# MiloniAtal/gato-python

Hardware: AMD Instinct MI355X
Metric: PCG iterations/s (higher is better)
Workload: dtype f64; 1 GPU; iiwa_14_7_k50_f64; STATE_SIZE=14, CONTROL_SIZE=7, KNOT_POINTS=50, max_iters=100, pcg_kernel=resident (one workgroup, mixed 2/1 rows per lane), pcg_workgroups=1, pcg_threads=512

## Files before the change

gato_python_amd/csrc/gato_assembly.hip:

```cpp
#include "gato_common.h"
#include "gato_gj.h"

namespace gato {
namespace {

constexpr int WAVE = 64;

template <typename T, int S, int C>
__global__ void add_rho_kernel(const T *__restrict__ G_in, T rho, T *__restrict__ Gd, size_t n_per_sys, int B)
{
    constexpr int SS = S * S, CC = C * C;
    const size_t total = n_per_sys * B;
    for (size_t i = (size_t)blockIdx.x * blockDim.x + threadIdx.x; i < total; i += (size_t)gridDim.x * blockDim.x) {
        const size_t w = (i % n_per_sys) % (SS + CC);
        const bool diag = w < SS ? (w % (S + 1) == 0) : ((w - SS) % (C + 1) == 0);
        Gd[i] = G_in[i] + (diag ? rho : (T)0);
    }
}

__device__ __forceinline__ void wave_sync() { __syncthreads(); }

template <typename T>
__device__ __forceinline__ void copy_in(T *dst, const T *__restrict__ src, int n, int lane)
{
// ... 306 lines not shown
    static constexpr int n = S + C, SS = S * S, CC = C * C, SC = S * C;
    static constexpr int Q = 0;
    static constexpr int R = Q + 3 * SS;
    static constexpr int AB = R + 3 * CC;
    static constexpr int PHI = AB + 2 * (SS + SC);
    static constexpr int BR = PHI + 2 * SS;
    static constexpr int TH = BR + 2 * SC;
    static constexpr int TT = TH + 2 * SS;
    static constexpr int VQ = TT + 2 * SS;
    static constexpr int VV = VQ + 2 * S + C;
    static constexpr int ELEMS = (VV + 3 * S + 3) / 4 * 4;
    static constexpr int PTR_G = 3 * n + 1, PTR_C = 2 * S + 1;
    static constexpr size_t BYTES = sizeof(T) * ELEMS + sizeof(int) * (PTR_G + PTR_C);
};

__device__ __forceinline__ int row_of_entry(const int *ptr, int nrows, int e)
{
    int lo = 0, hi = nrows;
    while (hi - lo > 1) {
        const int mid = (lo + hi) >> 1;
        if (ptr[mid] <= e) lo = mid; else hi = mid;
    }
    return lo;
}

template <typename T, int S, int C, int NT>
__global__ __launch_bounds__(NT, (GatherWaves<T, S>::v)) void gather_kernel(const int *__restrict__ G_row, const int *__restrict__ G_col,
                                                    const T *__restrict__ G_val, const int *__restrict__ C_row,
                                                    const int *__restrict__ C_col, const T *__restrict__ C_val, int K, T rho,
                                                    T *__restrict__ Gd, T *__restrict__ Cd, T *__restrict__ Ginv, BatchStride bs)
{
    constexpr int n = S + C, SS = S * S, CC = C * C, SC = S * C, ABS = SS + SC;
    static_assert(NT % WAVE == 0, "whole waves");
    __shared__ T blk[SS + CC + ABS];
    __shared__ int sPtrG[n + 1], sPtrC[S + 1];
    constexpr int NSLOT = SS + CC + ABS;
    __shared__ unsigned smask[(NSLOT + 31) / 32];
    __shared__ int sown[NSLOT];
    __shared__ int s_coll;
    T *sQ = blk, *sR = blk + SS, *sAB = blk + SS + CC;
    const int tid = threadIdx.x, lane = tid & 63, wave = tid >> 6;
    G_val += blockIdx.y * bs.nnzG; C_val += blockIdx.y * bs.nnzC;
    Gd += blockIdx.y * bs.g; Cd += blockIdx.y * bs.c;
    if (Ginv) Ginv += blockIdx.y * bs.g;
    for (int k = bs.k_lo + blockIdx.x; k < bs.k_hi; k += gridDim.x) {
        const bool last = k == K - 1;
// ... 52 lines not shown
                for (int t = tid; t < nG + nC; t += NT) {
                    const int colv = t < nG ? G_col[eG0 + t] : C_col[eC0 + (t - nG)];
                    const T valv = t < nG ? G_val[eG0 + t] : C_val[eC0 + (t - nG)];
                    T v;
                    const int sl = slot_of(t, colv, valv, v);
                    if (sl < 0) continue;
                    if (pass == 0) atomicMax(&sown[sl], t);
                    else if (sown[sl] == t) blk[sl] = v;
                }
                __syncthreads();
            }
        }
        __syncthreads();
        const size_t gk = (size_t)k * (SS + CC);
        for (int i = tid; i < SS + (last ? 0 : CC); i += NT) Gd[gk + i] = blk[i];
        if (!last) for (int i = tid; i < ABS; i += NT) Cd[(size_t)k * ABS + i] = sAB[i];
        if (Ginv) {
            if (wave == 0) invert_to<T, S>(sQ, Ginv + gk, lane, (T)1);
            if (wave == (NT > WAVE ? 1 : 0) && !last) invert_to<T, C>(sR, Ginv + gk + SS, lane, (T)1);
        }
    }
}

template <typename T, int S, int C, int NT>
__global__ __launch_bounds__(NT) void assemble_kernel(AsmArgs a, int K, BatchStride bs)
{
    typedef AsmLds<T, S, C> L;
    constexpr int n = S + C, SS = S * S, CC = C * C, SC = S * C, NW = NT / WAVE, ABS = SS + SC;
    static_assert(NW >= 6, "six inversions run side by side");
    constexpr int TILES = ((S + 15) / 16) * ((S + 15) / 16);
    extern __shared__ __align__(16) unsigned char lds_raw[];
    T *lds = (T *)lds_raw;
    T *sQ = lds + L::Q, *sR = lds + L::R, *sAB = lds + L::AB, *sPhi = lds + L::PHI, *sBR = lds + L::BR;
    T *sTh = lds + L::TH, *sT = lds + L::TT, *sq = lds + L::VQ, *sv = lds + L::VV;
    int *sPtrG = (int *)(lds + L::ELEMS), *sPtrC = sPtrG + L::PTR_G;
    constexpr int NSLOT = 3 * SS + 3 * CC + 2 * ABS;
    __shared__ unsigned smask[(NSLOT + 31) / 32];
    __shared__ int sown[NSLOT];
    __shared__ int s_coll;
    const int tid = threadIdx.x, lane = tid & 63, wave = tid >> 6;
    const int sys = blockIdx.y;
    const T *g = (const T *)a.g + sys * bs.n, *c = (const T *)a.c + sys * bs.sk;
    T *Gd = (T *)a.Gd + sys * bs.g, *Cd = (T *)a.Cd + sys * bs.c, *Ginv = (T *)a.Ginv + sys * bs.g;
    T *Sbd = (T *)a.Sbd + sys * bs.bd, *Pbd = (T *)a.Pbd + sys * bs.bd, *gamma = (T *)a.gamma + sys * bs.sk;
    const T rho = (T)a.rho;
    T *const iS = (T *)a.imgS, *const iP = (T *)a.imgP;
    const size_t ild = (size_t)a.img_ld;
    auto imS = [&](int kk, int b, int r, int cc, T v) { if (iS) iS[(size_t)(b * S + cc) * ild + (size_t)kk * S + r] = v; };
    auto imP = [&](int kk, int b, int r, int cc, T v) { if (iP) iP[(size_t)(b * S + cc) * ild + (size_t)kk * S + r] = v; };
    T *sQk = sQ + 2 * SS, *sRk = sR + 2 * CC, *sQm = sQ + SS, *sRm = sR + CC, *sQmm = sQ, *sRmm = sR;
    T *sA1 = sAB + ABS, *sB1 = sA1 + SS, *sA0 = sAB, *sB0 = sAB + SS;
    T *sPhi1 = sPhi + SS, *sPhi0 = sPhi, *sBR1 = sBR + SC, *sBR0 = sBR, *sTh1 = sTh + SS, *sTh0 = sTh;
    int n_stamp = 0;
    auto stamp = [&]() {
        if (a.stamps && blockIdx.x == (K > 2 ? 2 : 0) && sys == 0 && tid == 0) a.stamps[n_stamp++] = __builtin_amdgcn_s_memrealtime();
    };
    stamp();

    for (int k = blockIdx.x; k < K; k += gridDim.x) {
        const bool first = k == 0, last = k == K - 1;
        const bool full0 = k >= 2;
        const size_t gk = (size_t)k * (SS + CC);
        const size_t cm = first ? 0 : (size_t)(k - 1) * ABS;
        T *Sk = Sbd + (size_t)k * 3 * SS, *Pk = Pbd + (size_t)k * 3 * SS;
        static_assert(2 * S + C <= NT && S <= NT - 2 * WAVE, "one element of g and of c per thread");
        const int n_gq = first ? S : n + S;
        const int i_cq = first ? tid : tid - 2 * WAVE;
        const T gq = tid < n_gq ? g[(first ? 0 : (size_t)(k - 1) * n) + tid] : (T)0;
        const T cq = i_cq >= 0 && i_cq < S ? c[(size_t)k * S + i_cq] : (T)0;
        __syncthreads();
        if (a.mode == 0) {
            const T *G_val = (const T *)a.G_val + sys * bs.nnzG, *C_val = (const T *)a.C_val + sys * bs.nnzC;
            const int r0 = (k >= 2 ? k - 2 : 0) * n, nrG = k * n + (last ? S : n) - r0;
            const int c0 = (k >= 2 ? k - 1 : 1) * S, nrC = first ? 0 : (k + 1) * S - c0;
            static_assert(L::PTR_G <= NT && L::PTR_C <= NT, "one row pointer per thread");
            const int pG = tid <= nrG ? a.G_row[r0 + tid] : 0;
            const int pC = nrC && tid <= nrC ? a.C_row[c0 + tid] : 0;
            for (int i = tid; i < 3 * SS + 3 * CC + 2 * ABS; i += NT) lds[i] = (T)0;
            for (int i = tid; i < (NSLOT + 31) / 32; i += NT) smask[i] = 0u;
            if (tid == 0) s_coll = 0;
            if (tid <= nrG) sPtrG[tid] = pG;
            if (nrC && tid <= nrC) sPtrC[tid] = pC;
            __syncthreads();
            const int eG0 = sPtrG[0], nG = sPtrG[nrG] - eG0;
            const int eC0 = nrC ? sPtrC[0] : 0, nC = nrC ? sPtrC[nrC] - eC0 : 0;
            auto slot_of = [&](int t, int colv, T valv, T &v) -> int {
                if (t < nG) {
                    const int row = r0 + row_of_entry(sPtrG, nrG, eG0 + t);
                    const int knot = row / n, isr = row - knot * n, qi = knot - (k - 2);
                    const int isc = colv % n;
                    v = valv + (colv == row ? rho : (T)0);
                    if (isc < S) return isr < S ? L::Q + qi * SS + isc * S + isr : -1;
                    return isr >= S ? L::R + qi * CC + (isc - S) * C + (isr - S) : -1;
                }
                const int row = c0 + row_of_entry(sPtrC, nrC, eC0 + (t - nG));
                const int br = row / S - 1, i = row - (br + 1) * S;
                v = valv;
                return colv / n <= br ? L::AB + (br - (k - 2)) * ABS + (colv % n) * S + i : -1;
            };
            constexpr int U = 4;
            for (int t0 = tid; t0 < nG + nC; t0 += NT * U) {
                int col[U];
                T val[U];
#pragma unroll
                for (int u = 0; u < U; ++u) {
                    const int t = t0 + u * NT;
                    if (t < nG) { col[u] = a.G_col[eG0 + t]; val[u] = G_val[eG0 + t]; }
                    else if (t < nG + nC) { col[u] = a.C_col[eC0 + (t - nG)]; val[u] = C_val[eC0 + (t - nG)]; }
                }
#pragma unroll
                for (int u = 0; u < U; ++u) {
                    const int t = t0 + u * NT;
                    if (t < nG + nC) {
                        T v;
                        const int sl = slot_of(t, col[u], val[u], v);
                        if (sl >= 0) {
                            lds[sl] = v;
                            const unsigned bit = 1u << (sl & 31);
                            if (atomicOr(&smask[sl >> 5], bit) & bit) s_coll = 1;
                        }
                    }
                }
            }
            __syncthreads();
            if (s_coll) {
                for (int i = tid; i < NSLOT; i += NT) sown[i] = -1;
                __syncthreads();
                for (int pass = 0; pass < 2; ++pass) {
                    for (int t = tid; t < nG + nC; t += NT) {
                        const int colv = t < nG ? a.G_col[eG0 + t] : a.C_col[eC0 + (t - nG)];
                        const T valv = t < nG ? G_val[eG0 + t] : C_val[eC0 + (t - nG)];
                        T v;
                        const int sl = slot_of(t, colv, valv, v);
                        if (sl < 0) continue;
                        if (pass == 0) atomicMax(&sown[sl], t);
                        else if (sown[sl] == t) lds[sl] = v;
                    }
                    __syncthreads();
                }
            }
        } else {
            const T *Gin = a.mode == 2 ? (const T *)a.G_val + sys * bs.g : Gd;
            const T r2 = a.mode == 2 ? rho : (T)0;
#pragma unroll
            for (int qi = 0; qi < 3; ++qi) {
                const int knot = k - 2 + qi;
                if (knot < 0) continue;
                const size_t go = (size_t)knot * (SS + CC);
                for (int i = tid; i < SS; i += NT) sQ[qi * SS + i] = Gin[go + i] + ((i % (S + 1) == 0) ? r2 : (T)0);
                if (knot < K - 1)
                    for (int i = tid; i < CC; i += NT) sR[qi * CC + i] = Gin[go + SS + i] + ((i % (C + 1) == 0) ? r2 : (T)0);
                if (qi < 2 && knot < K - 1) copy_nt<NT>(sAB + qi * ABS, Cd + (size_t)knot * ABS, ABS, tid);
            }
        }
        if (tid < n_gq) sq[tid] = gq;
        __syncthreads();
        stamp();
        if (a.mode != 1) {
            for (int i = tid; i < SS; i += NT) Gd[gk + i] = sQk[i];
            if (!last) for (int i = tid; i < CC; i += NT) Gd[gk + SS + i] = sRk[i];
            if (a.mode == 0 && !first) for (int i = tid; i < ABS; i += NT) Cd[cm + i] = sA1[i];
        }
        if (first) for (int i = tid; i < SS; i += NT) { Pk[SS + i] = -sQk[i]; imP(0, 1, i % S, i / S, -sQk[i]); }
        if (k == 1) for (int i = tid; i < SS; i += NT) sTh0[i] = -sQm[i];
        __syncthreads();
        {
            T *mS = wave == 0 ? sQk : wave == 1 ? sQm : sQmm, *mC = wave == 5 ? sRk : wave == 2 ? sRm : sRmm;
            if (wave == 0 || (wave == 1 && !first) || (wave == 3 && full0)) invert_to<T, S>(mS, mS, lane, (T)1);
            else if ((wave == 5 && !last) || (wave == 2 && !first) || (wave == 4 && full0)) invert_to<T, C>(mC, mC, lane, (T)1);
        }
        __syncthreads();
        stamp();
        for (int i = tid; i < SS; i += NT) Ginv[gk + i] = sQk[i];
        if (!last) for (int i = tid; i < CC; i += NT) Ginv[gk + SS + i] = sRk[i];
        if (first) {
            if (wave == 0) mv<T, S, S>(sv, sQk, sq, lane);
            for (int i = tid; i < SS; i += NT) {
                Sk[i] = (T)0;
                Sk[SS + i] = -sQk[i];
// ... 170 lines not shown
    bs.stair_follows = d.stair_follows;
    if (!have_inverses) {
        const int nblk = (2 * (d.hi() - d.lo()) + 3) / 4;
        hipLaunchKernelGGL((invert_G_kernel<T, S, C>), dim3(nblk < 8192 ? nblk : 8192, d.B), dim3(256), 0, st, Gd, Ginv, d.K,
                           batch_stride(d));
        GATO_HIP_CHECK(hipGetLastError());
    }
    hipLaunchKernelGGL((schur_kernel<T, S, C>), dim3(knot_grid(d.hi() - d.lo()), d.B), dim3(WAVE), 0, st, Gd, Ginv, Cd, g, c, d.K,
                       Sbd, Pbd, gamma, bs);
    GATO_HIP_CHECK(hipGetLastError());
    return GATO_OK;
}

template <typename T, int S, int C>
int launch_assemble(const Dims &d, const AsmArgs &a, hipStream_t st)
{
    constexpr int NT = 512;
    typedef AsmLds<T, S, C> L;
    if (L::BYTES > 48 * 1024) {
        static bool attr_set[64] = {};
        int dev = 0;
        GATO_HIP_CHECK(hipGetDevice(&dev));
        if (dev < 0 || dev >= 64 || !attr_set[dev]) {
            GATO_HIP_CHECK(hipFuncSetAttribute((const void *)assemble_kernel<T, S, C, NT>,
                                               hipFuncAttributeMaxDynamicSharedMemorySize, (int)L::BYTES));
            if (dev >= 0 && dev < 64) attr_set[dev] = true;
        }
    }
    const int gx = d.K < (1 << 20) ? d.K : (1 << 20);
    hipLaunchKernelGGL((assemble_kernel<T, S, C, NT>), dim3(gx, d.B), dim3(NT), L::BYTES, st, a, d.K, batch_stride(d));
    GATO_HIP_CHECK(hipGetLastError());
    return GATO_OK;
}

template <typename T, int S, int C>
int launch_form_ss(const Dims &d, const T *Sbd, T *Pbd, hipStream_t st)
{
    hipLaunchKernelGGL((ss_kernel<T, S>), dim3(knot_grid(d.hi() - d.lo()), d.B), dim3(WAVE), 0, st, Sbd, Pbd, d.K, batch_stride(d));
    GATO_HIP_CHECK(hipGetLastError());
    return GATO_OK;
}

template <typename T, int S, int C>
int launch_point_jacobi(const Dims &d, const T *Sbd, T *Pbd, hipStream_t st)
{
    const size_t total = d.bd();
    const int blocks = (int)((total + 255) / 256 < 4096 ? (total + 255) / 256 : 4096);
    hipLaunchKernelGGL((point_jacobi_kernel<T, S>), dim3(blocks, d.B), dim3(256), 0, st, Sbd, Pbd, d.K, batch_stride(d));
    GATO_HIP_CHECK(hipGetLastError());
    return GATO_OK;
}

template <typename T, int S, int C>
// ... 37 lines not shown
```

gato_python_amd/csrc/gato_capi.hip:

```cpp
#include <cmath>
#include <cstdarg>
#include <cstdlib>
#include "gato_solver.h"

namespace gato {

static thread_local char g_err[512] = "";

void set_error(const char *fmt, ...)
{
    va_list ap;
    va_start(ap, fmt);
    vsnprintf(g_err, sizeof(g_err), fmt, ap);
    va_end(ap);
}

}

using namespace gato;

bool solver_usable(const gato_solver *s, const char *entry, const char *unsupported)
{
    if (!s) set_error("%s: null solver", entry);
    else if (s->cl.on || s->cl.local) set_error("%s: the solver is a cluster rank; sharded %s are not supported", entry, unsupported);
// ... 103 lines not shown
        return GATO_ENODEV;
    }
    GATO_HIP_CHECK(hipSetDevice(device));
    gato_solver *s = new gato_solver();
    memset(s, 0, sizeof(*s));
    s->d = Dims{S, C, K};
    s->d.B = B;
    s->dtype = dtype;
    s->device = device;
    s->esz = dtype == GATO_F32 ? 4 : 8;
    s->ops = ops;
    hipDeviceProp_t p;
    GATO_HIP_CHECK(hipGetDeviceProperties(&p, device));
    s->num_cus = p.multiProcessorCount;
    ops->pcg_plan(&s->plan);
    s->pcg_mode = GATO_PCG_AUTO;
    s->xcd_pack = -1;
    s->xcd_sel = -1;
    s->wave_pub = 1;
    s->dpp_rows = -1;
    s->pcg_semi = -1;
    s->timeout_ms = 2000;
    s->cluster_flat = 1;

    const Dims &d = s->d;
    const size_t e = s->esz;
    const int max_groups = 4096;
    size_t off = 0;
    auto take = [&](size_t bytes) { size_t o = off; off += align_up(bytes ? bytes : 8); return o; };
    const size_t o_status = take(64);
    const int slot_g = pcg_slot_granules(S, (int)e) > pcg_slot_granules_cg1(S, (int)e) ? pcg_slot_granules(S, (int)e)
                                                                                        : pcg_slot_granules_cg1(S, (int)e);
    const size_t o_slots = take((size_t)2 * 256 * slot_g * 8);
    s->slots_bytes = (size_t)2 * 256 * slot_g * 8;
    const size_t nb = (size_t)B;
    const size_t o_G = take(d.g_dense() * e * nb), o_C = take(d.c_dense() * e * nb), o_Gi = take(d.g_dense() * e * nb);
    const size_t o_S = take(d.bd() * e * nb), o_P = take(d.bd() * e * nb), o_gam = take(d.sk() * e * nb);
    const size_t o_lam = take(d.sk() * e * nb), o_dz = take(d.N() * e * nb);
    const size_t o_its = take(sizeof(int) * nb);
    const size_t o_vec = take(6 * d.sk() * e);
    const size_t o_part = take((size_t)4 * max_groups * e), o_scal = take(64 * 8), o_done = take(64);
    const size_t o_gh = take((size_t)8 * S * e);
    const size_t o_hist = take(sizeof(double) * (GATO_ETA_HIST_MAX + 1));
    const size_t o_xtab = take(sizeof(void *) * GATO_MAX_RANKS);
    const long long rows = (long long)K * S;
    const bool img = B == 1 && ((s->plan.pair_threads > 0 && rows <= 2ll * s->plan.pair_threads) || (s->plan.mixed_rows > 0 && rows <= s->plan.mixed_rows));
// ... 32 lines not shown
}

extern "C" int gato_solver_destroy(gato_solver *s)
{
    if (!s) return GATO_OK;
    (void)hipSetDevice(s->device);
    gato_cluster_destroy(s);
    if (s->ev_pcg0) (void)hipEventDestroy(s->ev_pcg0);
    if (s->ev_pcg1) (void)hipEventDestroy(s->ev_pcg1);
    if (s->ev_cal0) (void)hipEventDestroy(s->ev_cal0);
    if (s->ev_cal1) (void)hipEventDestroy(s->ev_cal1);
    for (int i = 0; i < 4; ++i)
        if (s->ev_stage[i]) (void)hipEventDestroy(s->ev_stage[i]);
    if (s->arena) (void)hipFree(s->arena);
    if (s->rhs_ws) (void)hipFree(s->rhs_ws);
    if (s->qp_ws) (void)hipFree(s->qp_ws);
    if (s->pol_ws) (void)hipFree(s->pol_ws);
    if (s->cross_ws) (void)hipFree(s->cross_ws);
    if (s->cross_rhs_ws) (void)hipFree(s->cross_rhs_ws);
    if (s->in_arena) (void)hipFree(s->in_arena);
    for (int i = 0; i < 2; ++i)
        if (s->host_ev[i]) (void)hipEventDestroy(s->host_ev[i]);
    if (s->pin) (void)hipHostFree(s->pin);
    delete s;
    return GATO_OK;
}

extern "C" void *gato_solver_buffer(gato_solver *s, int which)
{
    switch (which) {
        case 0: return s->G_dense;
        case 1: return s->C_dense;
        case 2: return s->Ginv;
        case 3: return s->Sbd;
        case 4: return s->Pbd;
        case 5: return s->gamma;
        case 6: return s->lambda;
        case 7: return s->dz;
        case 8: return s->iters;
        case 9: return (unsigned long long *)s->sw.scalars + 8;
        case 10: return s->eta_hist;
        case 11: return s->rhs_ws;
        case 12: return s->qp_pcg_total;
        case 13: case 14: case 15: case 16: {
            if (!s->cross_ws) return nullptr;
            const size_t e = s->esz, nb = (size_t)s->d.B;
            size_t off = 0;
            if (which > 13) off += align_up(s->d.g_dense() * e * nb);
            if (which > 14) off += align_up(s->d.c_dense() * e * nb);
            if (which > 15) off += align_up((size_t)(s->d.K - 1) * s->d.S * s->d.C * e * nb);
            return s->cross_ws + off;
        }
        default: return nullptr;
    }
}

extern "C" int gato_solver_set_option(gato_solver *s, const char *name, int value)
{
    if (!strcmp(name, "pcg_mode")) s->pcg_mode = value;
    else if (!strcmp(name, "pcg_threads")) s->pcg_threads = value;
    else if (!strcmp(name, "pcg_groups")) s->pcg_groups = value;
    else if (!strcmp(name, "asm_mode")) s->asm_mode = value;
    else if (!strcmp(name, "pcg_semi")) s->pcg_semi = value;
    else if (!strcmp(name, "pcg_epoch")) s->pcg_epoch = (unsigned)value;
    else if (!strcmp(name, "cluster_epoch")) s->cl.xepoch = (unsigned)value;
    else if (!strcmp(name, "stamp_asm")) s->stamp_asm = value;
    else if (!strcmp(name, "stamp_pcg")) s->stamp_pcg = value;
    else if (!strcmp(name, "ablate")) s->ablate = value;
    else if (!strcmp(name, "no_single_lds")) s->no_single_lds = value;
    else if (!strcmp(name, "no_pair")) s->no_pair = value;
    else if (!strcmp(name, "wave_pub")) s->wave_pub = value;
    else if (!strcmp(name, "dpp_rows")) s->dpp_rows = value;
    else if (!strcmp(name, "pcg_variant")) s->pcg_variant = value;
    else if (!strcmp(name, "record_eta")) s->record_eta = value;
    else if (!strcmp(name, "xcd_pack")) s->xcd_pack = value;
    else if (!strcmp(name, "xcd_sel")) s->xcd_sel = value < 0 ? -1 : (value & 7);
    else if (!strcmp(name, "true_warm_start")) s->true_warm_start = value;
    else if (!strcmp(name, "timeout_ms")) s->timeout_ms = value > 0 ? value : 2000;
    else if (!strcmp(name, "max_workgroups")) s->max_workgroups = value;
    else if (!strcmp(name, "no_fuse_dz")) s->no_fuse_dz = value;
    else if (!strcmp(name, "no_image")) s->no_image = value;
    else if (!strcmp(name, "qp_cross_unfused")) s->qp_cross_unfused = value;
    else if (!strcmp(name, "coop_launch")) s->coop_launch = value;
    else if (!strcmp(name, "cluster_flat")) s->cluster_flat = value;
    else if (!strcmp(name, "knot_lo") || !strcmp(name, "knot_hi")) {
        if (value < 0 || value > s->d.K) { set_error("%s = %d is outside [0, %d]", name, value, s->d.K); return GATO_EINVAL; }
        (name[5] == 'l' ? s->d.k_lo : s->d.k_hi) = value;
    }
    else if (!strcmp(name, "precon_mode")) {
// ... 28 lines not shown

extern "C" int gato_last_stage_ms(gato_solver *s, float *ms)
{
    if (!s->time_stages || !s->ev_stage[0]) { set_error("last_stage_ms: option time_stages is off"); return GATO_EINVAL; }
    GATO_HIP_CHECK(hipEventSynchronize(s->ev_stage[3]));
    for (int i = 0; i < 3; ++i) GATO_HIP_CHECK(hipEventElapsedTime(ms + i, s->ev_stage[i], s->ev_stage[i + 1]));
    return GATO_OK;
}

extern "C" int gato_solver_get_option(gato_solver *s, const char *name, int *value)
{
    if (!strcmp(name, "pcg_mode")) *value = s->pcg_mode;
    else if (!strcmp(name, "pcg_threads")) *value = s->pcg_threads;
    else if (!strcmp(name, "pcg_groups")) *value = s->pcg_groups;
    else if (!strcmp(name, "last_groups")) *value = s->last_groups;
    else if (!strcmp(name, "last_threads")) *value = s->last_threads;
    else if (!strcmp(name, "last_mode")) *value = s->last_mode;
    else if (!strcmp(name, "last_pair")) *value = s->last_pair;
    else if (!strcmp(name, "last_dpp")) *value = s->last_dpp;
    else if (!strcmp(name, "last_xcd_sel")) *value = s->last_xcd_sel;
    else if (!strcmp(name, "last_variant")) *value = s->last_variant;
    else if (!strcmp(name, "asm_mode")) *value = s->asm_mode;
    else if (!strcmp(name, "last_asm_fused")) *value = s->last_asm_fused;
    else if (!strcmp(name, "last_image")) *value = s->last_image;
    else if (!strcmp(name, "last_semi")) *value = s->last_semi;
    else if (!strcmp(name, "last_fallback")) *value = s->last_fallback;
    else if (!strcmp(name, "last_dz_fused")) *value = s->dz_fused;
    else if (!strcmp(name, "last_cluster_flat")) *value = s->cl.on ? s->cl.last_flat : 0;
    else if (!strcmp(name, "timeout_ms")) *value = s->timeout_ms;
    else if (!strcmp(name, "precon_mode")) *value = s->precon_mode;
    else if (!strcmp(name, "cluster_mem_kind")) *value = s->cl.on ? s->cl.mem_kind : -1;
    else if (!strcmp(name, "num_cus")) *value = s->num_cus;
    else if (!strcmp(name, "batch")) *value = s->d.B;
    else if (!strcmp(name, "rhs_reserved")) *value = s->rhs_R;
    else if (!strcmp(name, "assembly_valid")) *value = s->as.valid;
    else if (!strcmp(name, "assembly_gen")) *value = (int)s->as.gen;
    else if (!strcmp(name, "true_warm_start")) *value = s->true_warm_start;
    else if (!strcmp(name, "max_semi_knots"))
        *value = s->plan.semi_threads > 0 ? (s->plan.semi_threads / s->d.S + s->plan.semi_rows * s->plan.semi_threads / s->d.S) * (s->num_cus < 256 ? s->num_cus : 256) : 0;
    else if (!strcmp(name, "max_resident_knots")) *value = s->plan.max_knots_per_wg * (s->num_cus < 256 ? s->num_cus : 256);
    else { set_error("unknown option %s", name); return GATO_EINVAL; }
    return GATO_OK;
}

static bool owned(const gato_solver *s, const void *p)
{
    const char *q = (const char *)p;
// ... 43 lines not shown
```

gato_python_amd/csrc/gato_common.h:

```cpp
#pragma once
#include <hip/hip_runtime.h>

#include <cstddef>
#include <cstdint>
#include <cstdio>
#include <cstring>

#include "../../include/gato_hip.h"

#ifndef GATO_EXTRA_SHAPES
#define GATO_EXTRA_SHAPES(X)
#endif
#ifndef GATO_SHAPES
#define GATO_SHAPES(X) X(2, 1) X(14, 7) X(32, 16) X(4, 2) X(6, 3) X(12, 6) GATO_EXTRA_SHAPES(X)
#endif

#define GATO_MAX_RANKS 8

namespace gato {

void set_error(const char *fmt, ...);

__device__ __forceinline__ float fmaT(float a, float b, float c) { return __builtin_fmaf(a, b, c); }
__device__ __forceinline__ double fmaT(double a, double b, double c) { return __builtin_fma(a, b, c); }
// ... 176 lines not shown

struct PcgPlan {
    int max_threads;
    int max_knots_per_wg;
    int single_max_threads;
    int pair_threads;
    int mixed_rows, mixed_threads;
    int semi_threads;
    int semi_rows;
    int nores_threads;
    int nores_rows;
    int dpp_lanes;
};

template <typename T, int S, int C>
int launch_convert(const Dims &d, const int *G_row, const int *G_col, const T *G_val, const int *C_row,
                   const int *C_col, const T *C_val, T rho, T *Gd, T *Cd, T *Ginv ,
                   hipStream_t st);
template <typename T, int S, int C>
int launch_add_rho(const Dims &d, const T *G_in, T rho, T *Gd, hipStream_t st);
template <typename T, int S, int C>
int launch_form_schur(const Dims &d, const T *Gd, const T *Cd, const T *g, const T *c, T *Sbd, T *Pbd,
                      T *gamma, T *Ginv, bool have_inverses, hipStream_t st);
struct AsmArgs {
    int mode;
    const int *G_row, *G_col, *C_row, *C_col;
    const void *G_val, *C_val;
    double rho;
    const void *g, *c;
    void *Gd, *Cd, *Ginv, *Sbd, *Pbd, *gamma;
    void *imgS, *imgP;
    int img_ld;
    unsigned long long *stamps;
};
template <typename T, int S, int C>
int launch_assemble(const Dims &d, const AsmArgs &a, hipStream_t st);

template <typename T, int S, int C>
int launch_form_ss(const Dims &d, const T *Sbd, T *Pbd, hipStream_t st);
template <typename T, int S, int C>
int launch_point_jacobi(const Dims &d, const T *Sbd, T *Pbd, hipStream_t st);
template <typename T, int S, int C>
int launch_compute_dz(const Dims &d, const T *Ginv, const T *Cd, const T *g, const T *lambda, T *dz,
                      hipStream_t st);
template <typename T, int S, int C>
int launch_rhs_gamma(const Dims &d, int R, const T *Ginv, const T *Cd, const T *Sbd, const T *g, const T *c, T *gamma,
                     hipStream_t st);
template <typename T, int S, int C>
int launch_grad_blocks(const Dims &d, const T *dz, const T *lam, const T *a, const T *beta, T *Gbar, T *Cbar, hipStream_t st);
template <typename T, int S, int C>
int launch_grad_csr(const Dims &d, const int *G_row, const int *G_col, int nnzG, const int *C_row, const int *C_col, int nnzC,
                    const T *dz, const T *lam, const T *a, const T *beta, T *Gbar, T *Cbar, hipStream_t st);
#define GATO_QP_NSLOT 10
struct QpArgs {
    const void *G, *Cd, *g, *c, *lo, *hi;
    void *Gp;
// ... 234 lines not shown
```

gato_python_amd/csrc/gato_solve.hip:

```cpp
#include "gato_solver.h"

static int assemble(gato_solver *s, const AsmInput &in, const void *d_g, const void *d_c, double rho, hipStream_t st)
{
    int rc;
    const int mode = in.mode;
    s->d.k_lo = s->d.k_hi = 0;
    const long long knots = (long long)s->d.K * s->d.B;
    const bool stair = s->precon_mode == GATO_PRECON_STAIR;
    const bool fused = !in.have_inv && stair && (s->asm_mode == 2 || (s->asm_mode == 0 && knots <= 2ll * s->num_cus));
    s->last_asm_fused = fused;
    s->img_fresh = 0;
    s->as.valid = 0;
    s->as.img = 0;
    if (!fused) {
        if (in.have_inv) rc = GATO_OK;
        else if (mode == 0) {
            if (s->d.B > 1 && (s->d.nnzG <= 0 || s->d.nnzC <= 0)) return gato_convert(s, in.G_row, in.G_col, in.G_val, in.C_row, in.C_col, in.C_val, rho, s->G_dense, s->C_dense, st);
            rc = s->ops->convert(s->d, in.G_row, in.G_col, in.G_val, in.C_row, in.C_col, in.C_val, rho, s->G_dense, s->C_dense, s->Ginv, st);
        } else rc = s->ops->add_rho(s->d, in.G_val, rho, s->G_dense, st);
        if (rc) return rc;
        s->d.stair_follows = s->precon_mode == GATO_PRECON_STAIR;
        rc = s->ops->form_schur(s->d, s->G_dense, in.C_dense, d_g, d_c, s->Sbd, s->Pbd, s->gamma, s->Ginv, mode == 0 || in.have_inv, st);
        s->d.stair_follows = 0;
        if (rc) return rc;
        if (s->precon_mode == GATO_PRECON_BLOCK_JACOBI) return GATO_OK;
        if (s->precon_mode == GATO_PRECON_POINT_JACOBI) return s->ops->point_jacobi(s->d, s->Sbd, s->Pbd, st);
        return gato_form_ss(s, s->Sbd, s->Pbd, st);
    }
    if (mode == 0 && s->d.B > 1 && (s->d.nnzG <= 0 || s->d.nnzC <= 0)) {
        set_error("a batched solver needs the per-system nnz (gato_linsys_device_batched, or options batch_nnz_G / batch_nnz_C)");
        return GATO_EINVAL;
    }
    AsmArgs a;
    memset(&a, 0, sizeof(a));
    a.mode = mode;
    a.G_row = in.G_row; a.G_col = in.G_col; a.G_val = in.G_val; a.C_row = in.C_row; a.C_col = in.C_col; a.C_val = in.C_val;
    a.rho = rho; a.g = d_g; a.c = d_c;
    a.Gd = s->G_dense; a.Cd = const_cast<void *>(in.C_dense); a.Ginv = s->Ginv; a.Sbd = s->Sbd; a.Pbd = s->Pbd; a.gamma = s->gamma;
    a.stamps = s->stamp_asm ? (unsigned long long *)s->sw.scalars + 8 : nullptr;
    if (s->imgS && !s->no_image && s->d.B == 1) {
        a.imgS = s->imgS; a.imgP = s->imgP; a.img_ld = s->img_ld;
        s->img_fresh = 1;
        s->as.img = 1;
    }
    return s->ops->assemble(s->d, a, st);
}

int whole_solve(gato_solver *s, const PcgOpts &o, const AsmInput &in, const void *d_g, const void *d_c, double exit_tol,
                int max_iters, double rho, void *lam, void *dz, hipStream_t st)
{
    int rc;
    const bool ts = s->time_stages != 0 && !in.have_inv;
    if (ts) GATO_HIP_CHECK(hipEventRecord(s->ev_stage[0], st));
    if ((rc = assemble(s, in, d_g, d_c, rho, st))) return rc;
    if (ts) GATO_HIP_CHECK(hipEventRecord(s->ev_stage[1], st));
    s->lc = {1, s->Sbd, s->Pbd, s->gamma, in.C_dense, d_g, lam, dz, exit_tol, max_iters};
    s->fz = {s->Ginv, in.C_dense, d_g, dz};
    rc = pcg_systems(s, o, s->Sbd, s->Pbd, s->gamma, lam, exit_tol, max_iters, s->iters, st);
    s->fz = {nullptr, nullptr, nullptr, nullptr};
    s->img_fresh = 0;
    if (rc) return rc;
    if (ts) GATO_HIP_CHECK(hipEventRecord(s->ev_stage[2], st));
    if (!s->dz_fused && (rc = gato_compute_dz(s, s->Ginv, in.C_dense, d_g, lam, dz, st))) return rc;
    if (ts) GATO_HIP_CHECK(hipEventRecord(s->ev_stage[3], st));
    s->as = {1, in.C_dense, s->as.img, s->as.gen + 1};
    return GATO_OK;
}

// ... 184 lines not shown
```

gato_python_amd/csrc/gato_solver.h:

```cpp
#pragma once
#include <mutex>

#include "gato_common.h"

using namespace gato;

#define GATO_ETA_HIST_MAX 4096

struct gato_solver {
    Dims d;
    int dtype, device;
    size_t esz;
    const Ops *ops;
    int num_cus;
    int pcg_mode, pcg_threads, pcg_groups;
    int wave_pub;
    char *arena;
    size_t arena_bytes;
    void *G_dense, *C_dense, *Ginv, *Sbd, *Pbd, *gamma, *lambda, *dz;
    int *iters, *status;
    double *final_eta;
    unsigned long long *slots;
    PcgStreamWork sw;
    PcgPlan plan;
    char *in_arena;
// ... 65 lines not shown
    unsigned long long **cl_tab;
    struct {
        int valid;
        const void *Cd;
        int img;
        unsigned long long gen;
    } as;
    char *rhs_ws;
    size_t rhs_ws_bytes;
    int rhs_R;
    char *qp_ws;
    size_t qp_ws_bytes;
    int *qp_pcg_total;
    char *pol_ws;
    size_t pol_ws_bytes;
    char *cross_ws;
    size_t cross_ws_bytes;
    char *cross_rhs_ws;
    size_t cross_rhs_ws_bytes;
    struct {
        int valid;
        unsigned long long gen;
    } cross;
    int qp_cross_unfused;
};

inline size_t align_up(size_t x, size_t a = 256) { return (x + a - 1) / a * a; }

inline bool stream_is_capturing(hipStream_t st)
{
    hipStreamCaptureStatus cap = hipStreamCaptureStatusNone;
    if (hipStreamIsCapturing(st, &cap) != hipSuccess) (void)hipGetLastError();
    return cap != hipStreamCaptureStatusNone;
}

bool solver_usable(const gato_solver *s, const char *entry, const char *unsupported);

struct PcgGeometry { int groups, threads, kpw, pair, semi, dpp; bool cg1; };
struct PcgOpts { int mode, warm, stamp; };
inline PcgOpts pcg_opts(const gato_solver &s) { return PcgOpts{s.pcg_mode, s.true_warm_start, s.stamp_pcg}; }
bool plan_resident(const gato_solver &s, const PcgOpts &o, int K, int batch, bool plain_only, PcgGeometry *geo);
bool plan_cg1(const gato_solver &s, int K, PcgGeometry *geo);
bool plan_one_wg_each(const gato_solver &s, const PcgOpts &o, int n);
bool cluster_plan(const gato_solver &s, const PcgOpts &o, int rank, PcgGeometry *geo);
bool cluster_plan_cg1(const gato_solver &s, const PcgOpts &o, PcgGeometry *geo, int *flat_total, int *flat_base);
bool cluster_plan_flat(const gato_solver &s, const PcgOpts &o, int *flat_total, int *flat_base);
// ... 47 lines not shown
```

Baseline: 604,900 iterations/s.

## Cache precomputed CSR scatter plan for assembly across calls

Adds a one-time build kernel that precomputes, for each CSR entry of G and C, its destination slot in the per-knot LDS blocks, plus per-knot entry ranges. The assembly kernel then scatters values straight to LDS using that plan, skipping the binary row search and the duplicate-collision pass. The plan is keyed on the sparsity pointer addresses and checked against the live row pointers and columns, falling back to the old path and flagging it stale on a mismatch. It adds extra device memory and a 64-bit entry load per nonzero. The metric is PCG iterations/s, and assembly may not be inside the timed PCG loop.

```diff
diff --git a/gato_python_amd/csrc/gato_asm_scatter.h b/gato_python_amd/csrc/gato_asm_scatter.h
--- /dev/null
+++ b/gato_python_amd/csrc/gato_asm_scatter.h
@@ -0,0 +1,68 @@
+#pragma once
+#include <cstddef>
+
+namespace gato {
+
+struct AsmScatterKey {
+    const int *G_row, *G_col, *C_row, *C_col;
+    bool operator==(const AsmScatterKey &o) const { return G_row == o.G_row && G_col == o.G_col && C_row == o.C_row && C_col == o.C_col; }
+};
+
+struct AsmScatterState {
+    AsmScatterKey key;
+    unsigned gen;
+    int last;
+    unsigned last_gen;
+};
+
+enum AsmScatterAction {
+    ASM_SCATTER_NONE = 0,
+    ASM_SCATTER_USE,
+    ASM_SCATTER_BUILD,
+};
+
+inline AsmScatterAction asm_scatter_decide(const AsmScatterState &s, const AsmScatterKey &cur, unsigned stale_word, bool enabled, bool capturing)
+{
+    if (!enabled) return ASM_SCATTER_NONE;
+    const bool mine = s.gen != 0 && s.key == cur;
+    if (mine && stale_word != s.gen) return ASM_SCATTER_USE;
+    if (capturing) return mine ? ASM_SCATTER_USE : ASM_SCATTER_NONE;
+    return ASM_SCATTER_BUILD;
+}
+
+inline void asm_scatter_note(AsmScatterState &s, const AsmScatterKey &cur, AsmScatterAction act)
+{
+    if (act == ASM_SCATTER_BUILD) {
+        s.key = cur;
+        s.gen = s.gen + 1 ? s.gen + 1 : 1;
+    }
+    s.last = act != ASM_SCATTER_NONE;
+    s.last_gen = s.gen;
+}
+
+inline int asm_scatter_last(const AsmScatterState &s, unsigned stale_word)
+{
+    if (!s.last) return 0;
+    return stale_word == s.last_gen ? -1 : 1;
+}
+
+struct AsmScatterLayout { size_t tab, rowG, rowC, ent, bytes; int capG, capC; };
+inline AsmScatterLayout asm_scatter_layout(int S, int C, int K)
+{
+    AsmScatterLayout l;
+    const size_t rowsG = (size_t)(S + C) * K - C, rowsC = (size_t)S * K;
+    l.capG = (int)(2 * (size_t)(S * S + C * C) * K + 64);
+    l.capC = (int)(2 * (size_t)(S * S + S * C) * K + S + 64);
+    size_t off = 0;
+    auto take = [&](size_t ints) { const size_t o = off; off += (ints * sizeof(int) + 255) / 256 * 256; return o; };
+    l.tab = take((size_t)4 * K); l.rowG = take(rowsG + 1); l.rowC = take(rowsC + 1);
+    l.ent = take(2 * ((size_t)l.capG + l.capC));
+    l.bytes = off;
+    return l;
+}
+inline bool asm_scatter_fits(int S, int C, int K)
+{
+    return (long long)(K + 1) * (2 * S * S + C * C + S * C) < 0x7fffffffll && 2ll * (S * S + S * C) * K + S + 64 < 0x7fffffffll;
+}
+
+}
diff --git a/gato_python_amd/csrc/gato_assembly.hip b/gato_python_amd/csrc/gato_assembly.hip
--- a/gato_python_amd/csrc/gato_assembly.hip
+++ b/gato_python_amd/csrc/gato_assembly.hip
@@ -352,6 +352,87 @@
         if (ptr[mid] <= e) lo = mid; else hi = mid;
     }
     return lo;
+}
+
+template <int S, int C>
+__device__ __forceinline__ int g_entry_local(int row, int colv, int &knot)
+{
+    constexpr int n = S + C, SS = S * S;
+    knot = row / n;
+    const int isr = row - knot * n, isc = colv % n;
+    if (isc < S) return isr < S ? isc * S + isr : -1;
+    return isr >= S ? SS + (isc - S) * C + (isr - S) : -1;
+}
+template <int S, int C>
+__device__ __forceinline__ int c_entry_local(int row, int colv, int &br)
+{
+    constexpr int n = S + C, SS = S * S, CC = C * C;
+    br = row / S - 1;
+    const int i = row - (br + 1) * S;
+    return colv / n <= br ? SS + CC + (colv % n) * S + i : -1;
+}
+template <typename T, int S, int C>
+__device__ __forceinline__ int asm_place(int k, int knot, int local)
+{
+    typedef AsmLds<T, S, C> L;
+    constexpr int SS = S * S, CC = C * C, ABS = SS + S * C;
+    const int qi = knot - (k - 2);
+    if (local < SS) return L::Q + qi * SS + local;
+    if (local < SS + CC) return L::R + qi * CC + (local - SS);
+    return L::AB + qi * ABS + (local - SS - CC);
+}
+template <typename U> using global_ptr = const U __attribute__((address_space(1))) *;
+template <typename U>
+__device__ __forceinline__ global_ptr<U> uniform_value(const U *p)
+{
+    asm volatile("" : "+s"(p));
+    return (global_ptr<U>)p;
+}
+template <int S, int C>
+__device__ __forceinline__ void asm_rows(int k, int K, int &r0, int &nrG, int &c0, int &nrC)
+{
+    constexpr int n = S + C;
+    r0 = (k >= 2 ? k - 2 : 0) * n; nrG = k * n + (k == K - 1 ? S : n) - r0;
+    c0 = (k >= 2 ? k - 1 : 1) * S; nrC = k == 0 ? 0 : (k + 1) * S - c0;
+}
+
+template <int S, int C>
+__global__ __launch_bounds__(256) void asm_scatter_build_kernel(const int *__restrict__ G_row, const int *__restrict__ G_col,
+                                                                const int *__restrict__ C_row, const int *__restrict__ C_col,
+                                                                AsmScatter p, int K)
+{
+    constexpr int n = S + C, LOCAL = 2 * S * S + C * C + S * C;
+    const int rowsG = n * K - C, rowsC = S * K;
+    int *tab = const_cast<int *>(p.tab), *rowG = const_cast<int *>(p.rowG), *rowC = const_cast<int *>(p.rowC);
+    for (int i = blockIdx.x * blockDim.x + threadIdx.x; i < rowsG + rowsC + K; i += gridDim.x * blockDim.x) {
+        if (i < rowsG + rowsC) {
+            const bool isG = i < rowsG;
+            const int row = isG ? i : i - rowsG;
+            const int *ptr = isG ? G_row : C_row, *col = isG ? G_col : C_col;
+            unsigned long long *ent = const_cast<unsigned long long *>(p.ent) + (isG ? 0 : p.capG);
+            const int cap = isG ? p.capG : p.capC;
+            const int b = ptr[row], e = ptr[row + 1];
+            (isG ? rowG : rowC)[row] = b;
+            if (row == (isG ? rowsG : rowsC) - 1) (isG ? rowG : rowC)[row + 1] = e;
+            for (int j = b < 0 ? 0 : b; j < e && j < cap; ++j) {
+                const int colv = col[j];
+                int knot, kn2;
+                int local = isG ? g_entry_local<S, C>(row, colv, knot) : c_entry_local<S, C>(row, colv, knot);
+                for (int j2 = j + 1; local >= 0 && j2 < e; ++j2)
+                    if ((isG ? g_entry_local<S, C>(row, col[j2], kn2) : c_entry_local<S, C>(row, col[j2], kn2)) == local) local = -1;
+                const unsigned rec = local < 0 ? ASM_SCATTER_DROPPED : (unsigned)(knot * LOCAL + local) | (isG && colv == row ? ASM_SCATTER_DIAG : 0u);
+                ent[j] = (unsigned long long)rec << 32 | (unsigned)colv;
+            }
+        } else {
+            const int k = i - rowsG - rowsC;
+            int r0, nrG, c0, nrC;
+            asm_rows<S, C>(k, K, r0, nrG, c0, nrC);
+            const int eG0 = G_row[r0], nG = G_row[r0 + nrG] - eG0;
+            const int eC0 = nrC ? C_row[c0] : 0, nC = nrC ? C_row[c0 + nrC] - eC0 : 0;
+            const bool fits = eG0 >= 0 && nG >= 0 && eG0 + nG <= p.capG && eC0 >= 0 && nC >= 0 && eC0 + nC <= p.capC;
+            tab[4 * k] = eG0; tab[4 * k + 1] = fits ? nG : -1; tab[4 * k + 2] = eC0; tab[4 * k + 3] = nC;
+        }
+    }
 }
 
 template <typename T, int S, int C, int NT>
@@ -450,7 +531,7 @@
     }
 }
 
-template <typename T, int S, int C, int NT>
+template <typename T, int S, int C, int NT, bool PLAN>
 __global__ __launch_bounds__(NT) void assemble_kernel(AsmArgs a, int K, BatchStride bs)
 {
     typedef AsmLds<T, S, C> L;
@@ -479,9 +560,17 @@
     T *sQk = sQ + 2 * SS, *sRk = sR + 2 * CC, *sQm = sQ + SS, *sRm = sR + CC, *sQmm = sQ, *sRmm = sR;
     T *sA1 = sAB + ABS, *sB1 = sA1 + SS, *sA0 = sAB, *sB0 = sAB + SS;
     T *sPhi1 = sPhi + SS, *sPhi0 = sPhi, *sBR1 = sBR + SC, *sBR0 = sBR, *sTh1 = sTh + SS, *sTh0 = sTh;
+    __shared__ int s_stale;
     int n_stamp = 0;
+    const bool stamping = a.stamps && blockIdx.x == (K > 2 ? 2 : 0) && sys == 0 && tid == 0;
     auto stamp = [&]() {
-        if (a.stamps && blockIdx.x == (K > 2 ? 2 : 0) && sys == 0 && tid == 0) a.stamps[n_stamp++] = __builtin_amdgcn_s_memrealtime();
+        if (stamping) a.stamps[n_stamp++] = __builtin_amdgcn_s_memrealtime();
+    };
+    auto stamp_gather = [&](int i, bool landed) {
+        if (PLAN && stamping) {
+            if (landed) asm volatile("s_waitcnt vmcnt(0)" ::: "memory");
+            a.stamps[5 + i] = __builtin_amdgcn_s_memrealtime();
+        }
     };
     stamp();
 
@@ -496,12 +585,73 @@
         const int i_cq = first ? tid : tid - 2 * WAVE;
         const T gq = tid < n_gq ? g[(first ? 0 : (size_t)(k - 1) * n) + tid] : (T)0;
         const T cq = i_cq >= 0 && i_cq < S ? c[(size_t)k * S + i_cq] : (T)0;
+        constexpr int UP = S <= 16 ? 4 : 8;
+        constexpr int LOCAL = 2 * SS + CC + SC;
+        int r0, nrG, c0, nrC;
+        asm_rows<S, C>(k, K, r0, nrG, c0, nrC);
+        bool planned = false, gathered = false;
+        int pl_eG0 = 0, pl_nG = 0, pl_eC0 = 0, pl_nC = 0, pl_col[UP], pl_ptr[4];
+        unsigned long long pl_ent[UP];
+        T pl_val[UP];
+        bool pl_bad = false;
+        const T *G_val = (const T *)a.G_val + sys * bs.nnzG, *C_val = (const T *)a.C_val + sys * bs.nnzC;
+        struct { global_ptr<int> colG, colC; global_ptr<T> valG, valC; global_ptr<unsigned long long> ent; int capG; } pp = {};
+        auto plan_load = [&](int t0) {
+#pragma unroll
+            for (int u = 0; u < UP; ++u) {
+                const int t = min(t0 + u * NT, pl_nG + pl_nC - 1);
+                const bool isG = t < pl_nG;
+                const int e = isG ? pl_eG0 + t : pl_eC0 + (t - pl_nG);
+                pl_col[u] = (isG ? pp.colG : pp.colC)[e]; pl_val[u] = (isG ? pp.valG : pp.valC)[e];
+                pl_ent[u] = pp.ent[isG ? e : pp.capG + e];
+            }
+        };
+        auto plan_scatter = [&](int t0) {
+#pragma unroll
+            for (int u = 0; u < UP; ++u) {
+                const int t = t0 + u * NT;
+                if (t < pl_nG + pl_nC) {
+                    pl_bad |= (unsigned)pl_col[u] != (unsigned)pl_ent[u];
+                    const unsigned rec = (unsigned)(pl_ent[u] >> 32) & ~ASM_SCATTER_DIAG;
+                    if (rec != ASM_SCATTER_DROPPED) {
+                        const int knot = (int)(rec / (unsigned)LOCAL), local = (int)(rec - (unsigned)knot * LOCAL);
+                        const T v = t < pl_nG ? pl_val[u] + ((pl_ent[u] >> 63) ? rho : (T)0) : pl_val[u];
+                        lds[asm_place<T, S, C>(k, knot, local)] = v;
+                    }
+                }
+            }
+        };
+        if (PLAN && a.mode == 0 && a.sp.ent) {
+            typedef const int __attribute__((address_space(4))) *uniform_ints;
+            uniform_ints tab = (uniform_ints)(a.sp.tab + 4 * (size_t)k);
+            pl_eG0 = tab[0]; pl_nG = tab[1]; pl_eC0 = tab[2]; pl_nC = tab[3];
+            planned = pl_nG >= 0;
+            pp = {uniform_value(a.G_col), uniform_value(a.C_col), uniform_value(G_val), uniform_value(C_val), uniform_value(a.sp.ent), a.sp.capG};
+        }
+        if (PLAN && planned) {
+            static_assert(L::PTR_G <= NT && L::PTR_C <= NT, "one row pointer per thread");
+            const int iG = r0 + min(tid, nrG), iC = c0 + min(tid, nrC);
+            pl_ptr[0] = a.G_row[iG]; pl_ptr[1] = a.sp.rowG[iG]; pl_ptr[2] = a.C_row[iC]; pl_ptr[3] = a.sp.rowC[iC];
+            if (pl_nG + pl_nC > 0) plan_load(tid);
+            for (int i = tid; i < 3 * SS + 3 * CC + 2 * ABS; i += NT) lds[i] = (T)0;
+            if (tid == 0) s_stale = 0;
+        }
         __syncthreads();
-        if (a.mode == 0) {
-            const T *G_val = (const T *)a.G_val + sys * bs.nnzG, *C_val = (const T *)a.C_val + sys * bs.nnzC;
-            const int r0 = (k >= 2 ? k - 2 : 0) * n, nrG = k * n + (last ? S : n) - r0;
-            const int c0 = (k >= 2 ? k - 1 : 1) * S, nrC = first ? 0 : (k + 1) * S - c0;
-            static_assert(L::PTR_G <= NT && L::PTR_C <= NT, "one row pointer per thread");
+        if (PLAN && planned) {
+            stamp_gather(0, false);
+            stamp_gather(1, true);
+            pl_bad = pl_ptr[0] != pl_ptr[1] || pl_ptr[2] != pl_ptr[3];
+            plan_scatter(tid);
+            for (int t0 = tid + NT * UP; t0 < pl_nG + pl_nC; t0 += NT * UP) { plan_load(t0); plan_scatter(t0); }
+            stamp_gather(2, false);
+            if (pl_bad) s_stale = 1;
+            if (tid < n_gq) sq[tid] = gq;
+            __syncthreads();
+            gathered = s_stale == 0;
+            if (!gathered && tid == 0) *a.sp.stale = a.sp.gen;
+        }
+        if (gathered) {
+        } else if (a.mode == 0) {
             const int pG = tid <= nrG ? a.G_row[r0 + tid] : 0;
             const int pC = nrC && tid <= nrC ? a.C_row[c0 + tid] : 0;
             for (int i = tid; i < 3 * SS + 3 * CC + 2 * ABS; i += NT) lds[i] = (T)0;
@@ -512,19 +662,18 @@
             __syncthreads();
             const int eG0 = sPtrG[0], nG = sPtrG[nrG] - eG0;
             const int eC0 = nrC ? sPtrC[0] : 0, nC = nrC ? sPtrC[nrC] - eC0 : 0;
+            stamp_gather(0, false);
             auto slot_of = [&](int t, int colv, T valv, T &v) -> int {
+                int knot, local;
                 if (t < nG) {
                     const int row = r0 + row_of_entry(sPtrG, nrG, eG0 + t);
-                    const int knot = row / n, isr = row - knot * n, qi = knot - (k - 2);
-                    const int isc = colv % n;
+                    local = g_entry_local<S, C>(row, colv, knot);
                     v = valv + (colv == row ? rho : (T)0);
-                    if (isc < S) return isr < S ? L::Q + qi * SS + isc * S + isr : -1;
-                    return isr >= S ? L::R + qi * CC + (isc - S) * C + (isr - S) : -1;
+                } else {
+                    local = c_entry_local<S, C>(c0 + row_of_entry(sPtrC, nrC, eC0 + (t - nG)), colv, knot);
+                    v = valv;
                 }
-                const int row = c0 + row_of_entry(sPtrC, nrC, eC0 + (t - nG));
-                const int br = row / S - 1, i = row - (br + 1) * S;
-                v = valv;
-                return colv / n <= br ? L::AB + (br - (k - 2)) * ABS + (colv % n) * S + i : -1;
+                return local < 0 ? -1 : asm_place<T, S, C>(k, knot, local);
             };
             constexpr int U = 4;
             for (int t0 = tid; t0 < nG + nC; t0 += NT * U) {
@@ -536,6 +685,7 @@
                     if (t < nG) { col[u] = a.G_col[eG0 + t]; val[u] = G_val[eG0 + t]; }
                     else if (t < nG + nC) { col[u] = a.C_col[eC0 + (t - nG)]; val[u] = C_val[eC0 + (t - nG)]; }
                 }
+                if (t0 == tid) stamp_gather(1, true);
 #pragma unroll
                 for (int u = 0; u < U; ++u) {
                     const int t = t0 + u * NT;
@@ -550,6 +700,7 @@
                     }
                 }
             }
+            stamp_gather(2, false);
             __syncthreads();
             if (s_coll) {
                 for (int i = tid; i < NSLOT; i += NT) sown[i] = -1;
@@ -581,8 +732,10 @@
                 if (qi < 2 && knot < K - 1) copy_nt<NT>(sAB + qi * ABS, Cd + (size_t)knot * ABS, ABS, tid);
             }
         }
-        if (tid < n_gq) sq[tid] = gq;
-        __syncthreads();
+        if (!gathered) {
+            if (tid < n_gq) sq[tid] = gq;
+            __syncthreads();
+        }
         stamp();
         if (a.mode != 1) {
             for (int i = tid; i < SS; i += NT) Gd[gk + i] = sQk[i];
@@ -799,13 +952,24 @@
         int dev = 0;
         GATO_HIP_CHECK(hipGetDevice(&dev));
         if (dev < 0 || dev >= 64 || !attr_set[dev]) {
-            GATO_HIP_CHECK(hipFuncSetAttribute((const void *)assemble_kernel<T, S, C, NT>,
+            GATO_HIP_CHECK(hipFuncSetAttribute((const void *)assemble_kernel<T, S, C, NT, false>,
+                                               hipFuncAttributeMaxDynamicSharedMemorySize, (int)L::BYTES));
+            GATO_HIP_CHECK(hipFuncSetAttribute((const void *)assemble_kernel<T, S, C, NT, true>,
                                                hipFuncAttributeMaxDynamicSharedMemorySize, (int)L::BYTES));
             if (dev >= 0 && dev < 64) attr_set[dev] = true;
         }
     }
+    if (a.mode == 0 && a.sp.ent && a.sp.build) {
+        const long long work = (long long)(2 * S + C) * d.K + d.K;
+        hipLaunchKernelGGL((asm_scatter_build_kernel<S, C>), dim3((unsigned)((work + 255) / 256 < 4096 ? (work + 255) / 256 : 4096)), dim3(256),
+                           0, st, a.G_row, a.G_col, a.C_row, a.C_col, a.sp, d.K);
+        GATO_HIP_CHECK(hipGetLastError());
+    }
     const int gx = d.K < (1 << 20) ? d.K : (1 << 20);
-    hipLaunchKernelGGL((assemble_kernel<T, S, C, NT>), dim3(gx, d.B), dim3(NT), L::BYTES, st, a, d.K, batch_stride(d));
+    if (a.mode == 0 && a.sp.ent)
+        hipLaunchKernelGGL((assemble_kernel<T, S, C, NT, true>), dim3(gx, d.B), dim3(NT), L::BYTES, st, a, d.K, batch_stride(d));
+    else
+        hipLaunchKernelGGL((assemble_kernel<T, S, C, NT, false>), dim3(gx, d.B), dim3(NT), L::BYTES, st, a, d.K, batch_stride(d));
     GATO_HIP_CHECK(hipGetLastError());
     return GATO_OK;
 }
diff --git a/gato_python_amd/csrc/gato_capi.hip b/gato_python_amd/csrc/gato_capi.hip
--- a/gato_python_amd/csrc/gato_capi.hip
+++ b/gato_python_amd/csrc/gato_capi.hip
@@ -149,6 +149,7 @@
     s->pcg_semi = -1;
     s->timeout_ms = 2000;
     s->cluster_flat = 1;
+    s->asm_plan = 1;
 
     const Dims &d = s->d;
     const size_t e = s->esz;
@@ -227,6 +228,8 @@
     for (int i = 0; i < 2; ++i)
         if (s->host_ev[i]) (void)hipEventDestroy(s->host_ev[i]);
     if (s->pin) (void)hipHostFree(s->pin);
+    if (s->sp_mem) (void)hipFree(s->sp_mem);
+    if (s->sp_stale) (void)hipHostFree(s->sp_stale);
     delete s;
     return GATO_OK;
 }
@@ -256,6 +259,8 @@
             if (which > 15) off += align_up((size_t)(s->d.K - 1) * s->d.S * s->d.C * e * nb);
             return s->cross_ws + off;
         }
+        case 17: return s->imgS;
+        case 18: return s->imgP;
         default: return nullptr;
     }
 }
@@ -270,6 +275,7 @@
     else if (!strcmp(name, "pcg_epoch")) s->pcg_epoch = (unsigned)value;
     else if (!strcmp(name, "cluster_epoch")) s->cl.xepoch = (unsigned)value;
     else if (!strcmp(name, "stamp_asm")) s->stamp_asm = value;
+    else if (!strcmp(name, "asm_plan")) s->asm_plan = value;
     else if (!strcmp(name, "stamp_pcg")) s->stamp_pcg = value;
     else if (!strcmp(name, "ablate")) s->ablate = value;
     else if (!strcmp(name, "no_single_lds")) s->no_single_lds = value;
@@ -344,7 +350,10 @@
     else if (!strcmp(name, "last_variant")) *value = s->last_variant;
     else if (!strcmp(name, "asm_mode")) *value = s->asm_mode;
     else if (!strcmp(name, "last_asm_fused")) *value = s->last_asm_fused;
+    else if (!strcmp(name, "asm_plan")) *value = s->asm_plan;
+    else if (!strcmp(name, "last_asm_plan")) *value = asm_scatter_last(s->sp_state, s->sp_stale ? *(volatile unsigned *)s->sp_stale : 0u);
     else if (!strcmp(name, "last_image")) *value = s->last_image;
+    else if (!strcmp(name, "image_ld")) *value = s->imgS ? s->img_ld : 0;
     else if (!strcmp(name, "last_semi")) *value = s->last_semi;
     else if (!strcmp(name, "last_fallback")) *value = s->last_fallback;
     else if (!strcmp(name, "last_dz_fused")) *value = s->dz_fused;
diff --git a/gato_python_amd/csrc/gato_common.h b/gato_python_amd/csrc/gato_common.h
--- a/gato_python_amd/csrc/gato_common.h
+++ b/gato_python_amd/csrc/gato_common.h
@@ -222,6 +222,17 @@
 template <typename T, int S, int C>
 int launch_form_schur(const Dims &d, const T *Gd, const T *Cd, const T *g, const T *c, T *Sbd, T *Pbd,
                       T *gamma, T *Ginv, bool have_inverses, hipStream_t st);
+struct AsmScatter {
+    const int *tab;
+    const int *rowG, *rowC;
+    const unsigned long long *ent;
+    unsigned *stale;
+    unsigned gen;
+    int capG, capC;
+    int build;
+};
+constexpr unsigned ASM_SCATTER_DROPPED = 0x7fffffffu, ASM_SCATTER_DIAG = 0x80000000u;
+
 struct AsmArgs {
     int mode;
     const int *G_row, *G_col, *C_row, *C_col;
@@ -232,6 +243,7 @@
     void *imgS, *imgP;
     int img_ld;
     unsigned long long *stamps;
+    AsmScatter sp;
 };
 template <typename T, int S, int C>
 int launch_assemble(const Dims &d, const AsmArgs &a, hipStream_t st);
diff --git a/gato_python_amd/csrc/gato_solve.hip b/gato_python_amd/csrc/gato_solve.hip
--- a/gato_python_amd/csrc/gato_solve.hip
+++ b/gato_python_amd/csrc/gato_solve.hip
@@ -1,4 +1,26 @@
 #include "gato_solver.h"
+
+static int asm_scatter_alloc(gato_solver *s)
+{
+    if (s->sp_mem) return GATO_OK;
+    const AsmScatterLayout l = asm_scatter_layout(s->d.S, s->d.C, s->d.K);
+    GATO_HIP_CHECK(hipSetDevice(s->device));
+    if (!s->sp_stale) {
+        GATO_HIP_CHECK(hipHostMalloc((void **)&s->sp_stale, 64, hipHostMallocDefault));
+        *s->sp_stale = 0u;
+    }
+    GATO_HIP_CHECK(hipMalloc((void **)&s->sp_mem, l.bytes));
+    return GATO_OK;
+}
+
+static void asm_scatter_args(const gato_solver *s, bool build, AsmScatter *p)
+{
+    const AsmScatterLayout l = asm_scatter_layout(s->d.S, s->d.C, s->d.K);
+    const char *m = s->sp_mem;
+    p->tab = (const int *)(m + l.tab); p->rowG = (const int *)(m + l.rowG); p->rowC = (const int *)(m + l.rowC);
+    p->ent = (const unsigned long long *)(m + l.ent);
+    p->stale = s->sp_stale; p->gen = s->sp_state.gen; p->capG = l.capG; p->capC = l.capC; p->build = build;
+}
 
 static int assemble(gato_solver *s, const AsmInput &in, const void *d_g, const void *d_c, double rho, hipStream_t st)
 {
@@ -9,6 +31,7 @@
     const bool stair = s->precon_mode == GATO_PRECON_STAIR;
     const bool fused = !in.have_inv && stair && (s->asm_mode == 2 || (s->asm_mode == 0 && knots <= 2ll * s->num_cus));
     s->last_asm_fused = fused;
+    s->sp_state.last = 0;
     s->img_fresh = 0;
     s->as.valid = 0;
     s->as.img = 0;
@@ -38,12 +61,25 @@
     a.rho = rho; a.g = d_g; a.c = d_c;
     a.Gd = s->G_dense; a.Cd = const_cast<void *>(in.C_dense); a.Ginv = s->Ginv; a.Sbd = s->Sbd; a.Pbd = s->Pbd; a.gamma = s->gamma;
     a.stamps = s->stamp_asm ? (unsigned long long *)s->sw.scalars + 8 : nullptr;
+    AsmScatterAction act = ASM_SCATTER_NONE;
+    const AsmScatterKey key{in.G_row, in.G_col, in.C_row, in.C_col};
+    if (mode == 0) {
+        const bool capturing = stream_is_capturing(st);
+        const bool wanted = s->asm_plan >= 2 || (s->asm_plan == 1 && s->d.S <= 16);
+        const bool can = wanted && asm_scatter_fits(s->d.S, s->d.C, s->d.K) && (s->sp_mem || !capturing);
+        act = asm_scatter_decide(s->sp_state, key, s->sp_stale ? *(volatile unsigned *)s->sp_stale : 0u, can, capturing);
+        if (act != ASM_SCATTER_NONE && (rc = asm_scatter_alloc(s))) return rc;
+        asm_scatter_note(s->sp_state, key, act);
+        if (act != ASM_SCATTER_NONE) asm_scatter_args(s, act == ASM_SCATTER_BUILD, &a.sp);
+    }
     if (s->imgS && !s->no_image && s->d.B == 1) {
         a.imgS = s->imgS; a.imgP = s->imgP; a.img_ld = s->img_ld;
         s->img_fresh = 1;
         s->as.img = 1;
     }
-    return s->ops->assemble(s->d, a, st);
+    rc = s->ops->assemble(s->d, a, st);
+    if (rc && act == ASM_SCATTER_BUILD) s->sp_state.key = AsmScatterKey{};
+    return rc;
 }
 
 int whole_solve(gato_solver *s, const PcgOpts &o, const AsmInput &in, const void *d_g, const void *d_c, double exit_tol,
diff --git a/gato_python_amd/csrc/gato_solver.h b/gato_python_amd/csrc/gato_solver.h
--- a/gato_python_amd/csrc/gato_solver.h
+++ b/gato_python_amd/csrc/gato_solver.h
@@ -1,6 +1,7 @@
 #pragma once
 #include <mutex>
 
+#include "gato_asm_scatter.h"
 #include "gato_common.h"
 
 using namespace gato;
@@ -112,6 +113,10 @@
         int valid;
         unsigned long long gen;
     } cross;
+    int asm_plan;
+    AsmScatterState sp_state;
+    char *sp_mem;
+    unsigned *sp_stale;
     int qp_cross_unfused;
 };
 
```

After: 607,300 iterations/s (median of 6 runs). Within noise of the previous version (+0.4%).
